# snap-stanford/KGWAS

Measured on AMD Instinct MI355X. Metric: edges aggregated/sec (full fast-mode KG minibatch training; epoch time in config), higher is better.
Workload: dtype f32

## Files before the change

### kgwas_amd/csrc/kgw_dense_linear.h

```cpp
#pragma once

namespace {

constexpr int LBM = 128, LBN = 128, LBK = 32, LPAD = 33;

struct LinArgs {
    const float* X; int64_t ldx;
    const float* W; int64_t ldw;
    const float* bias;
    const float* mask;
    int64_t ldm;
    float* Y; int64_t ldy;
    int64_t rows; int K, N;
    int relu, w_kn;
    const int32_t* rows_dev;
};

__device__ __forceinline__ int64_t lin_rows_eff(const LinArgs& a) {
    if (!a.rows_dev) return a.rows;
    const int64_t r = *a.rows_dev;
    return r < 0 ? 0 : (r < a.rows ? r : a.rows);
}

__device__ __forceinline__ void lin_zero_padding(const LinArgs& a, int64_t rows_eff, int64_t tid, int64_t nthreads) {
// ... 1151 lines not shown
#pragma unroll
            for (int e = 0; e < 16; ++e) acc[t][e] = 0.f;
#pragma unroll
        for (int s_ = 0; s_ < 8; ++s_) {
            const f32x4 u = xa[2 * s_], v = xa[2 * s_ + 1];
            const float h[8] = {kgw_fxor(u.x, sgn), kgw_fxor(u.y, sgn), kgw_fxor(u.z, sgn), kgw_fxor(u.w, sgn),
                                kgw_fxor(v.x, sgn), kgw_fxor(v.y, sgn), kgw_fxor(v.z, sgn), kgw_fxor(v.w, sgn)};
            uint4 p1, p2, p3;
            kgw_split3x8(h, p1, p2, p3);
            const kgw_bf8 hb[3] = {__builtin_bit_cast(kgw_bf8, p1), __builtin_bit_cast(kgw_bf8, p2), __builtin_bit_cast(kgw_bf8, p3)};
            kgw_bf8 wa[3][4];
#pragma unroll
            for (int p = 0; p < 3; ++p)
#pragma unroll
                for (int jt = 0; jt < 4; ++jt) wa[p][jt] = __builtin_bit_cast(kgw_bf8, w2p[((s_ * 3 + p) * 4 + jt) * 64]);
            constexpr int TW[6] = {0, 2, 1, 0, 1, 0}, TH[6] = {2, 0, 1, 1, 0, 0};
#pragma unroll
            for (int t6 = 0; t6 < 6; ++t6)
#pragma unroll
                for (int jt = 0; jt < 4; ++jt)
                    acc[jt] = __builtin_amdgcn_mfma_f32_32x32x16_bf16(wa[TW[t6]][jt], hb[TH[t6]], acc[jt], 0, 0, 0);
            if (s_ == 3) {
                __builtin_amdgcn_sched_barrier(0);
#pragma unroll
                for (int qq = 0; qq < 8; ++qq) xa[qq] = *(const f32x4*)(xn + 4 * qq);
                __builtin_amdgcn_sched_barrier(0);
            }
        }
        if (!live) { mb[0] = 0u; mb[1] = 0u; }
        __builtin_amdgcn_sched_barrier(0);
#pragma unroll
        for (int qq = 8; qq < 16; ++qq) xa[qq] = *(const f32x4*)(xn + 4 * qq);
        __builtin_amdgcn_sched_barrier(0);
#pragma unroll
        for (int hh = 0; hh < 2; ++hh) {
#pragma unroll
            for (int t = 2 * hh; t < 2 * hh + 2; ++t)
#pragma unroll
                for (int g = 0; g < 4; ++g) {
                    const unsigned m4 = mb[t >> 1] >> (((t & 1) << 4) + 4 * g);
                    f32x4 v;
                    v.x = (m4 & 1u) ? kgw_fxor(acc[t][4 * g + 0], sgn) : 0.f; v.y = (m4 & 2u) ? kgw_fxor(acc[t][4 * g + 1], sgn) : 0.f;
                    v.z = (m4 & 4u) ? kgw_fxor(acc[t][4 * g + 2], sgn) : 0.f; v.w = (m4 & 8u) ? kgw_fxor(acc[t][4 * g + 3], sgn) : 0.f;
                    *(f32x4*)(Tw + li * TS2 + (t - 2 * hh) * 32 + 8 * g + 4 * lk) = v;
                    if (a.dZ && row < rows) *(f32x4*)(a.dZ + row * a.ldz + t * 32 + 8 * g + 4 * lk) = v;
                }
            __asm__ volatile("s_waitcnt lgkmcnt(0)" ::: "memory");
            if (PACK) {
                const bool neg = a.flip && ((tile / a.flip) & 1);
#pragma unroll
                for (int it = 0; it < 4; ++it) {
                    const int ntl = it & 1, j = it >> 1;
                    const float* tp = Tw + (16 * j + 8 * lk) * TS2 + 32 * ntl + li;
                    float x[8];
#pragma unroll
                    for (int i = 0; i < 8; ++i) x[i] = neg ? -tp[i * TS2] : tp[i * TS2];
                    uint4 p1, p2, p3;
                    kgw_split3x8(x, p1, p2, p3);
                    uint4* o = a.packed + (((int64_t)tile * 2 + j) * 3 * 4 + (2 * hh + ntl)) * 64 + lane;
                    o[0] = p1; o[4 * 64] = p2; o[8 * 64] = p3;
                }
            }
#pragma unroll
            for (int s2 = 0; s2 < 16; ++s2) {
                const float* tp = Tw + (2 * s2 + lk) * TS2 + li;
#pragma unroll
                for (int t = 0; t < 2; ++t)
                    accw[2 * hh + t] = __builtin_amdgcn_mfma_f32_32x32x2f32(xs[s2], tp[t * 32], accw[2 * hh + t], 0, 0, 0);
            }
            __asm__ volatile("s_waitcnt lgkmcnt(0)" ::: "memory");
        }
        mb[0] = 0u; mb[1] = 0u;
        KGW_MLPB_BITS(mvn, mb)
    }
#undef KGW_MLPB_BITS
    __syncthreads();
    float* R = lds;
#pragma unroll
    for (int t = 0; t < 4; ++t)
#pragma unroll
        for (int e = 0; e < 16; ++e) R[wave * 4096 + (t * 16 + e) * 64 + lane] = accw[t][e];
    __syncthreads();
    for (int f = tid; f < 4096; f += 256)
        a.part[(int64_t)blockIdx.x * 4096 + f] = (R[f] + R[4096 + f]) + (R[2 * 4096 + f] + R[3 * 4096 + f]);
}

__global__ void __launch_bounds__(1024) k_mlp2_bwd_fold(const float* __restrict__ part, int nblk, int K1, float* __restrict__ dW1,
                                                        int64_t ldw, float* __restrict__ db1) {
    __shared__ float sm[1024];
    const int fl = threadIdx.x & 63, g = threadIdx.x >> 6;
    const int f = blockIdx.x * 64 + fl;
    float s4[4] = {0.f, 0.f, 0.f, 0.f};
    int q = 0;
    for (int b = g; b < nblk; b += 16, ++q) s4[q & 3] += part[(int64_t)b * 4096 + f];
    sm[threadIdx.x] = (s4[0] + s4[1]) + (s4[2] + s4[3]);
    __syncthreads();
    if (g == 0) {
        float sv = 0.f;
#pragma unroll
        for (int k = 0; k < 16; k += 4) sv += (sm[k * 64 + fl] + sm[(k + 1) * 64 + fl]) + (sm[(k + 2) * 64 + fl] + sm[(k + 3) * 64 + fl]);
        const int lane = f & 63, e = (f >> 6) & 15, t = f >> 10;
        const int k = (e & 3) + 8 * (e >> 2) + 4 * (lane >> 5), col = 32 * t + (lane & 31);
        if (k < K1) dW1[(int64_t)col * ldw + k] = sv;
        else if (k == K1) db1[col] = sv;
    }
}

template <bool WKN, bool MASK>
__global__ void __launch_bounds__(256) __attribute__((amdgpu_waves_per_eu(2, 2))) k_linear_wreg_half(LinArgs a_) {
    extern __shared__ __attribute__((aligned(16))) float lds[];
    LinArgs a = a_;
    {
        const int64_t re = lin_rows_eff(a_);
        lin_zero_padding(a_, re, (int64_t)blockIdx.x * 256 + threadIdx.x, (int64_t)gridDim.x * 256);
        a.rows = re;
        if ((int64_t)blockIdx.x * 2 * 32 >= re) return;
    }
    float* Wl = lds;
    const int tid = threadIdx.x, lane = tid & 63, wave = tid >> 6;
    const int li = lane & 31, lk = lane >> 5;
    const int64_t tile = (int64_t)blockIdx.x * 2 + (wave >> 1);
    const int t0 = (wave & 1) * 2;
    const int64_t row = tile * 32 + li;
    const bool live = row < a.rows;
    const int64_t rc = live ? row : a.rows - 1;
    f32x4 xa[16];
    {
        const float* xp = a.X + rc * a.ldx + lk * 64;
#pragma unroll
        for (int q = 0; q < 16; ++q) xa[q] = *(const f32x4*)(xp + 4 * q);
    }
    f32x4 mv[2][4];
    if (MASK) {
        const float* mp = a.mask + rc * a.ldm + 4 * lk;
#pragma unroll
        for (int t = 0; t < 2; ++t)
#pragma unroll
            for (int g = 0; g < 4; ++g) mv[t][g] = *(const f32x4*)(mp + (t0 + t) * 32 + 8 * g);
    }
    {
        f32x4 wv[16];
#pragma unroll
        for (int it = 0; it < 16; ++it) {
            const int idx = tid + 256 * it;
            if (!WKN) wv[it] = *(const f32x4*)(a.W + (int64_t)(idx >> 5) * a.ldw + (idx & 31) * 4);
            else wv[it] = *(const f32x4*)(a.W + (int64_t)(idx & 127) * a.ldw + (idx >> 7) * 4);
        }
#pragma unroll
        for (int it = 0; it < 16; ++it) {
            const int idx = tid + 256 * it;
            if (!WKN) {
                *(f32x4*)(Wl + (idx >> 5) * WST + (idx & 31) * 4) = wv[it];
            } else {
                const int k = idx & 127, n4 = (idx >> 7) * 4;
                Wl[(n4 + 0) * WST + k] = wv[it].x; Wl[(n4 + 1) * WST + k] = wv[it].y;
                Wl[(n4 + 2) * WST + k] = wv[it].z; Wl[(n4 + 3) * WST + k] = wv[it].w;
            }
        }
    }
    if (tid < 128) Wl[128 * WST + tid] = a.bias ? a.bias[tid] : 0.f;
    __syncthreads();
    f32x4 bw[2][16];
#pragma unroll
    for (int t = 0; t < 2; ++t)
#pragma unroll
        for (int q = 0; q < 16; ++q) bw[t][q] = *(const f32x4*)(Wl + ((t0 + t) * 32 + li) * WST + lk * 64 + 4 * q);
// ... 135 lines not shown
        static KgwPerDevice attr3_set;
        if (attr3_set.need()) {
            KGW_HIP(hipFuncSetAttribute((const void*)k_mlp2_fwd3, hipFuncAttributeMaxDynamicSharedMemorySize, (int)lds3));
        }
        const int64_t nblk3 = ((rows + 31) / 32 + 7) / 8;
        k_mlp2_fwd3<<<(int)(nblk3 < 256 ? nblk3 : 256), 512, lds3, (hipStream_t)stream_>>>(a);
        KGW_LAUNCH_CHECK();
        return KGW_OK;
    }
    const int64_t nblk = ((rows + 31) / 32 + 3) / 4;
    k_mlp2_fwd<<<(int)(nblk < 256 ? nblk : 256), 256, lds, (hipStream_t)stream_>>>(a);
    KGW_LAUNCH_CHECK();
    return KGW_OK;
}

extern "C" int kgw_mlp2w_fwd(int32_t n_jobs, const float* const* src, const int32_t* const* ids, const int64_t* n_rows,
                             int64_t ldx, const float* W1, int64_t ldw1, const float* b1, const float* W2, int64_t ldw2,
                             const float* b2, float* Xg, float* H1, float* H2, int64_t ldo, kgw_stream_t stream_) {
    if (n_jobs <= 0) return KGW_OK;
    if (n_jobs > 4) return KGW_E_RANGE;
    if (!src || !ids || !n_rows || !W1 || !W2 || !Xg || !H1 || !H2) return KGW_E_NULL;
    if ((ldx & 3) || (ldw1 & 3) || (ldw2 & 3) || (ldo & 3) || !aligned16(W1) || !aligned16(W2) || !aligned16(Xg) || !aligned16(H1) ||
        !aligned16(H2))
        return KGW_E_UNSUPPORTED;
    Mlp2wArgs a{};
    a.n_jobs = n_jobs; a.ldx = ldx;
    a.row0[0] = 0;
    for (int j = 0; j < n_jobs; ++j) {
        if (!src[j] || !ids[j] || n_rows[j] < 0) return KGW_E_NULL;
        if (!aligned16(src[j])) return KGW_E_UNSUPPORTED;
        a.src[j] = src[j]; a.ids[j] = ids[j]; a.row0[j + 1] = a.row0[j] + n_rows[j];
    }
    a.rows = a.row0[n_jobs];
    if (a.rows == 0) return KGW_OK;
    a.W1 = W1; a.ldw1 = ldw1; a.b1 = b1; a.W2 = W2; a.ldw2 = ldw2; a.b2 = b2;
    a.Xg = Xg; a.H1 = H1; a.H2 = H2; a.ldo = ldo;
    const size_t lds = (size_t)(2 * 128 * WST + 256) * sizeof(float);
    static KgwPerDevice attr_once;
    if (attr_once.need()) {
        KGW_HIP(hipFuncSetAttribute((const void*)k_mlp2w_fwd, hipFuncAttributeMaxDynamicSharedMemorySize, (int)lds));
    }
    const int64_t ntiles = (a.rows + 31) / 32;
    k_mlp2w_fwd<<<(unsigned)((ntiles + 1) / 2), 256, lds, (hipStream_t)stream_>>>(a);
    KGW_LAUNCH_CHECK();
    return KGW_OK;
}

extern "C" int64_t kgw_mlp2_bwd_first_workspace_floats(int64_t rows) {
    int64_t nblk = ((rows + 31) / 32 + 3) / 4;
    if (nblk > 256) nblk = 256;
    if (nblk < 1) nblk = 1;
    return nblk * 4096;
}

static int mlp2_bwd_first(const float* dH2, int64_t ldd, const float* W2, int64_t ldw2, const float* H1, int64_t ldh1,
                          const float* X, int64_t ldx, int32_t K1, int64_t rows, const int32_t* rows_dev, float* dW1,
                          int64_t ldw1, float* db1, float* workspace, int64_t workspace_floats, const int32_t* in_ids,
                          float* dZ, int64_t ldz, kgw_stream_t stream_, KgwGradSrc* defer, void* packed = nullptr, int flip = 0) {
    if (!dH2 || !W2 || !H1 || !db1 || !workspace) return KGW_E_NULL;
    if (defer && K1 > 0 && ldw1 != K1) return KGW_E_UNSUPPORTED;
    if (rows <= 0 || K1 < 0) return KGW_E_RANGE;
    if (K1 > 0 && (!X || !dW1)) return KGW_E_NULL;
    if (dZ && ((ldz & 3) || !aligned16(dZ))) return KGW_E_UNSUPPORTED;
    if (K1 > 31 || (ldd & 3) || (ldw2 & 3) || (ldh1 & 3) || !aligned16(dH2) || !aligned16(W2) || !aligned16(H1)) return KGW_E_UNSUPPORTED;
    int64_t nblk = ((rows + 31) / 32 + 3) / 4;
    if (nblk > 256) nblk = 256;
    if (workspace_floats < nblk * 4096) return KGW_E_RANGE;
    Mlp2BwdArgs a{dH2, ldd, W2, ldw2, H1, ldh1, X, ldx, workspace, rows, K1, rows_dev, in_ids, dZ, ldz, (uint4*)packed, flip};
    const size_t lds = (size_t)(128 * WST + 4 * 32 * TST) * sizeof(float);
    static KgwPerDevice attr_once;
    if (attr_once.need()) {
        KGW_HIP(hipFuncSetAttribute((const void*)k_mlp2_bwd_first, hipFuncAttributeMaxDynamicSharedMemorySize, (int)lds));
    }
    hipStream_t st = (hipStream_t)stream_;
    static const bool split3 = !(getenv("KGW_MLP2_SPLIT") && getenv("KGW_MLP2_SPLIT")[0] == '0');
    if (packed && (!split3 || rows_dev || ((uintptr_t)packed & 15))) return KGW_E_UNSUPPORTED;
    if (split3) {
        const size_t lds3 = (size_t)M3_W2_U4 * 16 + (size_t)(4 * 32 * TS2) * sizeof(float);
        static KgwPerDevice attr3_set;
        if (attr3_set.need()) {
            KGW_HIP(hipFuncSetAttribute((const void*)k_mlp2_bwd_first3<false>, hipFuncAttributeMaxDynamicSharedMemorySize, (int)lds3));
            KGW_HIP(hipFuncSetAttribute((const void*)k_mlp2_bwd_first3<true>, hipFuncAttributeMaxDynamicSharedMemorySize, (int)lds3));
        }
        if (packed) k_mlp2_bwd_first3<true><<<(int)nblk, 256, lds3, st>>>(a);
        else k_mlp2_bwd_first3<false><<<(int)nblk, 256, lds3, st>>>(a);
    } else {
        k_mlp2_bwd_first<<<(int)nblk, 256, lds, st>>>(a);
    }
    KGW_LAUNCH_CHECK();
    if (defer) {
        defer[0] = KgwGradSrc{};
        defer[1] = KgwGradSrc{};
        if (K1 > 0) { defer[0].ws = workspace; defer[0].kind = KGW_GRAD_MLP2_W; defer[0].nblk = (int)nblk; defer[0].K1 = K1; }
        defer[1].ws = workspace; defer[1].kind = KGW_GRAD_MLP2_B; defer[1].nblk = (int)nblk; defer[1].K1 = K1;
        return KGW_OK;
    }
    k_mlp2_bwd_fold<<<4096 / 64, 1024, 0, st>>>(workspace, (int)nblk, K1, dW1, ldw1, db1);
    KGW_LAUNCH_CHECK();
    return KGW_OK;
}

extern "C" int kgw_mlp2_bwd_first(const float* dH2, int64_t ldd, const float* W2, int64_t ldw2, const float* H1, int64_t ldh1,
                                  const float* X, int64_t ldx, int32_t K1, int64_t rows, const int32_t* rows_dev, float* dW1,
                                  int64_t ldw1, float* db1, float* workspace, int64_t workspace_floats, const int32_t* in_ids,
                                  float* dZ, int64_t ldz, kgw_stream_t stream_) {
    return mlp2_bwd_first(dH2, ldd, W2, ldw2, H1, ldh1, X, ldx, K1, rows, rows_dev, dW1, ldw1, db1, workspace, workspace_floats,
                          in_ids, dZ, ldz, stream_, nullptr);
}

extern "C" int kgw_mlp2_bwd_first_partial(const float* dH2, int64_t ldd, const float* W2, int64_t ldw2, const float* H1,
                                          int64_t ldh1, const float* X, int64_t ldx, int32_t K1, int64_t rows,
                                          const int32_t* rows_dev, float* dW1, int64_t ldw1, float* db1, float* workspace,
                                          int64_t workspace_floats, const int32_t* in_ids, float* dZ, int64_t ldz, KgwGradSrc* src,
                                          kgw_stream_t stream_) {
    if (!src) return KGW_E_NULL;
    return mlp2_bwd_first(dH2, ldd, W2, ldw2, H1, ldh1, X, ldx, K1, rows, rows_dev, dW1, ldw1, db1, workspace, workspace_floats,
                          in_ids, dZ, ldz, stream_, src);
}

extern "C" int kgw_mlp2_bwd_first_packed(const float* dH2, int64_t ldd, const float* W2, int64_t ldw2, const float* H1,
                                         int64_t ldh1, const float* X, int64_t ldx, int32_t K1, int64_t rows, float* dW1,
                                         int64_t ldw1, float* db1, float* workspace, int64_t workspace_floats,
                                         const int32_t* in_ids, float* dZ, int64_t ldz, void* packed, int32_t flip, KgwGradSrc* src,
                                         kgw_stream_t stream_) {
    if (!packed) return KGW_E_NULL;
    if (flip < 0 || (flip & (flip - 1))) return KGW_E_RANGE;
    return mlp2_bwd_first(dH2, ldd, W2, ldw2, H1, ldh1, X, ldx, K1, rows, nullptr, dW1, ldw1, db1, workspace, workspace_floats,
                          in_ids, dZ, ldz, stream_, src, packed, flip);
}
```

### kgwas_amd/csrc/kgw_gemm3.hip

```cpp
#include "kgw_common.h"
#include "kgw_riders.h"
#include <stdlib.h>

typedef kgw_bf8 g3_bf8;
typedef __attribute__((ext_vector_type(16))) float g3_f16;
typedef __attribute__((ext_vector_type(4))) float g3_f4;
typedef __attribute__((ext_vector_type(4))) unsigned g3_u4;

static constexpr int G3_CH_U4 = 1536;
static constexpr int G3_FLIP = 16;
static int g3_flip() { return G3_FLIP; }
static constexpr int G3_MAX_ITEMS = 512;

template <bool KN>
__global__ void __launch_bounds__(256) k_g3_pack(const float* __restrict__ S, long lds_, int K, long kv, int vec, uint4* __restrict__ out, int flip) {
    const long t = (long)blockIdx.x * 256 + threadIdx.x;
    if (t >= (long)K * 16) return;
    const int lane = (int)(t & 63), nt = (int)((t >> 6) & 3), j = (int)((t >> 8) & 1);
    const long c = t >> 9;
    const int n = 32 * nt + (lane & 31);
    const long k0 = 32 * c + 16 * j + 8 * (lane >> 5);
    float x[8];
    if (KN) {
#pragma unroll
        for (int i = 0; i < 8; ++i) x[i] = k0 + i < kv ? S[(k0 + i) * lds_ + n] : 0.f;
    } else if (vec && k0 + 8 <= kv) {
        const float4 u = *(const float4*)(S + n * lds_ + k0), v = *(const float4*)(S + n * lds_ + k0 + 4);
        x[0] = u.x; x[1] = u.y; x[2] = u.z; x[3] = u.w; x[4] = v.x; x[5] = v.y; x[6] = v.z; x[7] = v.w;
    } else {
#pragma unroll
        for (int i = 0; i < 8; ++i) x[i] = k0 + i < kv ? S[n * lds_ + k0 + i] : 0.f;
    }
    if (flip && ((c / flip) & 1)) {
#pragma unroll
        for (int i = 0; i < 8; ++i) x[i] = -x[i];
    }
    uint4 p1, p2, p3;
    kgw_split3x8(x, p1, p2, p3);
    uint4* o = out + ((c * 2 + j) * 3 * 4 + nt) * 64 + lane;
    o[0] = p1; o[4 * 64] = p2; o[8 * 64] = p3;
}

struct G3Args {
    const float* A; long lda; int M, K;
    const uint4* Bp;
    float* ws;
    int nsplit, n_tiles, per_xcd, flip;
};

struct G3KArgs { G3Args a; G3Riders R; };
template <int MT, int NW = 4, bool IMG = false>
__global__ void __launch_bounds__(64 * NW, (8 / NW) / MT) k_g3_gemm(G3KArgs ka_) {
    const G3Args& a = ka_.a;
    constexpr int NT = 64 * NW, NB = G3_CH_U4 / NT;
    constexpr int NQ = 4 * MT;
    constexpr int AT = 256 * MT;
    __shared__ g3_u4 smB0[G3_CH_U4], smB1[G3_CH_U4];
    __shared__ g3_f4 smA0[IMG ? 1 : NW * AT], smA1[IMG ? 1 : NW * AT];
    const int tid = threadIdx.x, lane = tid & 63, wave = tid >> 6;
    if ((int)blockIdx.x >= a.per_xcd * 8) {
        const char* kseg = (const char*)__builtin_amdgcn_kernarg_segment_ptr();
        const G3Riders* R = (const G3Riders*)(kseg + __builtin_offsetof(G3KArgs, R));
        if (ka_.R.n_blocks) g3_param_riders<NW>(*R, (int)blockIdx.x - a.per_xcd * 8);
        return;
    }
    const int item = (int)(blockIdx.x & 7) * a.per_xcd + (int)(blockIdx.x >> 3);
    if ((int)(blockIdx.x >> 3) >= a.per_xcd || item >= a.n_tiles * a.nsplit) return;
    const int split = item / a.n_tiles, tile = item - split * a.n_tiles;
    const int nch = a.K >> 5;
    const int c0 = (int)((long)nch * split / a.nsplit), c1 = (int)((long)nch * (split + 1) / a.nsplit);
    const int nc = c1 - c0;
    const int row0 = tile * (32 * NW * MT) + wave * (32 * MT);

    const long cstep = a.lda > 0 ? 32 : 1024;
    const float* ap[NQ];
    int aw[NQ];
    if (IMG) {
        int t = row0 >> 5;
        t = t < ((a.M - 1) >> 5) ? t : ((a.M - 1) >> 5);
#pragma unroll
        for (int q = 0; q < NQ; ++q) {
            ap[q] = a.A + (long)t * -a.lda + (long)c0 * 1024 + (q * 64 + lane) * 4;
            aw[q] = 0;
        }
    } else
#pragma unroll
    for (int q = 0; q < NQ; ++q) {
        const int r = 8 * q + (lane >> 3);
        int row = row0 + r;
        row = row < a.M ? row : a.M - 1;
        ap[q] = a.lda ? a.A + (long)row * a.lda + (long)c0 * 32 + (lane & 7) * 4
                      : a.A + ((long)(row >> 5) * nch + c0) * 1024 + (row & 31) * 32 + (lane & 7) * 4;
        aw[q] = wave * AT + r * 8 + ((lane & 7) ^ ((r >> 1) & 7));
    }
    const int m = lane & 31, g = lane >> 5, sw = (m >> 1) & 7;
    const g3_u4* bp = (const g3_u4*)a.Bp + (long)c0 * G3_CH_U4 + tid;

    g3_f4 ra[NQ], rb[NQ];
    g3_u4 bs[NB];
    g3_f16 acc[MT][4];
#pragma unroll
    for (int mt = 0; mt < MT; ++mt)
#pragma unroll
        for (int nt = 0; nt < 4; ++nt)
#pragma unroll
            for (int i = 0; i < 16; ++i) acc[mt][nt][i] = 0.f;

    auto load_a = [&](g3_f4 (&r)[NQ], int c) {
#pragma unroll
        for (int q = 0; q < NQ; ++q) r[q] = __builtin_nontemporal_load((const g3_f4*)(ap[q] + (long)c * cstep));
    };
    auto store_a = [&](const g3_f4 (&r)[NQ], g3_f4* A) {
#pragma unroll
        for (int q = 0; q < NQ; ++q) A[aw[q]] = r[q];
    };
    auto load_b = [&](int c) {
#pragma unroll
        for (int i = 0; i < NB; ++i) bs[i] = bp[(long)c * G3_CH_U4 + i * NT];
    };
    auto store_b = [&](g3_u4* B) {
#pragma unroll
        for (int i = 0; i < NB; ++i) B[tid + i * NT] = bs[i];
    };
    auto compute = [&](const g3_f4* A_, const g3_u4* B_) {
        const g3_u4* B = B_ + lane;
        const g3_f4* A = A_ + wave * AT + m * 8;
#pragma unroll
        for (int j = 0; j < 2; ++j) {
            const int seg = 2 * (2 * j + g);
            g3_bf8 ap_[MT][3];
#pragma unroll
            for (int mt = 0; mt < MT; ++mt) {
                const g3_f4 u = A[mt * 256 + (seg ^ sw)], v = A[mt * 256 + ((seg + 1) ^ sw)];
                const float x[8] = {u[0], u[1], u[2], u[3], v[0], v[1], v[2], v[3]};
                uint4 p1, p2, p3;
                kgw_split3x8(x, p1, p2, p3);
                ap_[mt][0] = __builtin_bit_cast(g3_bf8, p1);
                ap_[mt][1] = __builtin_bit_cast(g3_bf8, p2);
                ap_[mt][2] = __builtin_bit_cast(g3_bf8, p3);
            }
            g3_bf8 b[3][4];
#pragma unroll
            for (int p = 0; p < 3; ++p)
#pragma unroll
                for (int nt = 0; nt < 4; ++nt) b[p][nt] = __builtin_bit_cast(g3_bf8, B[((j * 3 + p) * 4 + nt) * 64]);
            constexpr int TA[6] = {0, 2, 1, 0, 1, 0}, TB[6] = {2, 0, 1, 1, 0, 0};
#pragma unroll
            for (int t = 0; t < 6; ++t)
#pragma unroll
                for (int nt = 0; nt < 4; ++nt)
#pragma unroll
                    for (int mt = 0; mt < MT; ++mt)
                        acc[mt][nt] = __builtin_amdgcn_mfma_f32_32x32x16_bf16(ap_[mt][TA[t]], b[TB[t]][nt], acc[mt][nt], 0, 0, 0);
        }
    };

    auto compute_img = [&](g3_f4 (&r)[NQ], const g3_u4* B_, int cn) {
        const g3_u4* B = B_ + lane;
        g3_bf8 ap_[2][3];
#pragma unroll
        for (int j = 0; j < 2; ++j) {
            const g3_f4 u = r[2 * j], v = r[2 * j + 1];
            const float x[8] = {u[0], u[1], u[2], u[3], v[0], v[1], v[2], v[3]};
            uint4 p1, p2, p3;
            kgw_split3x8(x, p1, p2, p3);
            ap_[j][0] = __builtin_bit_cast(g3_bf8, p1);
            ap_[j][1] = __builtin_bit_cast(g3_bf8, p2);
            ap_[j][2] = __builtin_bit_cast(g3_bf8, p3);
        }
        load_a(r, cn);
#pragma unroll
        for (int j = 0; j < 2; ++j) {
            g3_bf8 b[3][4];
#pragma unroll
            for (int p = 0; p < 3; ++p)
#pragma unroll
                for (int nt = 0; nt < 4; ++nt) b[p][nt] = __builtin_bit_cast(g3_bf8, B[((j * 3 + p) * 4 + nt) * 64]);
            constexpr int TA[6] = {0, 2, 1, 0, 1, 0}, TB[6] = {2, 0, 1, 1, 0, 0};
#pragma unroll
            for (int t = 0; t < 6; ++t)
#pragma unroll
                for (int nt = 0; nt < 4; ++nt)
                    acc[0][nt] = __builtin_amdgcn_mfma_f32_32x32x16_bf16(ap_[j][TA[t]], b[TB[t]][nt], acc[0][nt], 0, 0, 0);
        }
    };

    auto flip = [&]() {
#pragma unroll
        for (int mt = 0; mt < MT; ++mt)
#pragma unroll
            for (int nt = 0; nt < 4; ++nt)
#pragma unroll
                for (int i = 0; i < 16; ++i) acc[mt][nt][i] = -acc[mt][nt][i];
    };
    const int last = nc - 1;
    if constexpr (IMG) {
        static_assert(MT == 1, "the operand image holds 32-row tiles");
        load_a(ra, 0);
        load_b(0);
        store_b(smB0);
        load_a(rb, min(1, last));
        load_b(min(1, last));
        __syncthreads();
        for (int c = 0; c < nc; c += 2) {
            store_b(smB1);
            load_b(min(c + 2, last));
            if (a.flip && c && !((c0 + c) & (a.flip - 1))) flip();
            compute_img(ra, smB0, min(c + 2, last));
            __syncthreads();
            if (c + 1 >= nc) break;
            store_b(smB0);
            load_b(min(c + 3, last));
            if (a.flip && !((c0 + c + 1) & (a.flip - 1))) flip();
            compute_img(rb, smB1, min(c + 3, last));
            __syncthreads();
        }
    } else {
        load_a(ra, 0);
        load_b(0);
        store_a(ra, smA0);
        store_b(smB0);
        load_a(ra, min(1, last));
        load_b(min(1, last));
        __syncthreads();
        for (int c = 0; c < nc; c += 2) {
            load_a(rb, min(c + 2, last));
            store_a(ra, smA1);
            store_b(smB1);
            load_b(min(c + 2, last));
            if (a.flip && c && !((c0 + c) & (a.flip - 1))) flip();
            compute(smA0, smB0);
            __syncthreads();
            if (c + 1 >= nc) break;
            load_a(ra, min(c + 3, last));
            store_a(rb, smA0);
            store_b(smB0);
            load_b(min(c + 3, last));
            if (a.flip && !((c0 + c + 1) & (a.flip - 1))) flip();
            compute(smA1, smB1);
            __syncthreads();
        }
    }

    float* wp = a.ws + ((long)split * a.M) * 128 + m;
    if (a.flip && (((c1 - 1) / a.flip) & 1)) flip();
#pragma unroll
    for (int mt = 0; mt < MT; ++mt)
#pragma unroll
        for (int r = 0; r < 16; ++r) {
            const int row = row0 + 32 * mt + 8 * (r >> 2) + 4 * g + (r & 3);
            if (row < a.M) {
#pragma unroll
                for (int nt = 0; nt < 4; ++nt) wp[(long)row * 128 + 32 * nt] = acc[mt][nt][r];
            }
        }
}

__global__ void __launch_bounds__(256) k_g3_reduce(const float* __restrict__ ws, int nsplit, long M, const float* __restrict__ bias,
                                                   int relu, float* __restrict__ out, long ldo, const int32_t* __restrict__ row_map,
                                                   float* __restrict__ out_rows, long ld_rows, long out_rows_n,
                                                   const int32_t* __restrict__ out_rows_real) {
    const long t = (long)blockIdx.x * 256 + threadIdx.x;
    if (out_rows_real) {
        const long real = *out_rows_real < 0 ? 0 : *out_rows_real;
        const long zr = real + (t >> 5);
        if (zr < out_rows_n) *(float4*)(out_rows + zr * ld_rows + 4 * (t & 31)) = make_float4(0.f, 0.f, 0.f, 0.f);
    }
    if (t >= M * 32) return;
    const long row = t >> 5;
    const int c4 = (int)(t & 31);
    const float4* w = (const float4*)ws + t;
    float4 s = w[0];
    for (int k = 1; k < nsplit; ++k) {
        const float4 v = w[(long)k * M * 32];
        s.x += v.x; s.y += v.y; s.z += v.z; s.w += v.w;
    }
    if (bias) {
        const float4 b = ((const float4*)bias)[c4];
        s.x += b.x; s.y += b.y; s.z += b.z; s.w += b.w;
    }
    if (relu) { s.x = fmaxf(s.x, 0.f); s.y = fmaxf(s.y, 0.f); s.z = fmaxf(s.z, 0.f); s.w = fmaxf(s.w, 0.f); }
    *(float4*)(out + row * ldo + 4 * c4) = s;
    if (row_map) {
        const int l = row_map[row];
        if (l >= 0) *(float4*)(out_rows + (long)l * ld_rows + 4 * c4) = s;
    }
}

__global__ void __launch_bounds__(256) k_g3_reduce_t(const float* __restrict__ ws, int nsplit, long M, float* __restrict__ out, long ldo) {
    __shared__ float tl[32][33];
    const int tid = threadIdx.x;
    const long r0 = (long)blockIdx.x * 32;
    const int cb = blockIdx.y * 32;
    {
        const int r = tid >> 3, c4 = tid & 7;
        float4 s = make_float4(0.f, 0.f, 0.f, 0.f);
        if (r0 + r < M) {
            const float4* w = (const float4*)ws + (r0 + r) * 32 + (cb >> 2) + c4;
            s = w[0];
            for (int k = 1; k < nsplit; ++k) {
                const float4 v = w[(long)k * M * 32];
                s.x += v.x; s.y += v.y; s.z += v.z; s.w += v.w;
            }
        }
        tl[r][4 * c4] = s.x; tl[r][4 * c4 + 1] = s.y; tl[r][4 * c4 + 2] = s.z; tl[r][4 * c4 + 3] = s.w;
    }
    __syncthreads();
    const int r = tid & 31;
    if (r0 + r < M) {
#pragma unroll
        for (int i = 0; i < 4; ++i) {
            const int col = (tid >> 5) + 8 * i;
            out[(long)(cb + col) * ldo + r0 + r] = tl[r][col];
        }
    }
}

static int g3_nw() { return 8; }

static int g3_splits(int64_t M, int64_t K) {
    const int rt = 32 * g3_nw();
    const int64_t tiles = (M + rt - 1) / rt, nch = K / 32;
    int64_t s = (G3_MAX_ITEMS * 4 / g3_nw()) / tiles;
    if (s > nch / 8) s = nch / 8;
    if (s > 16) s = 16;
    if (s < 1) s = 1;
    return (int)s;
}

static bool g3_a_ok(const float* A, int64_t lda, int64_t K) {
    if ((uintptr_t)A & 15) return false;
    if (lda < 0) return !(-lda % 1024) && -lda >= K / 32 * 1024;
    return !(lda & 3);
}

static void g3_gemm_launch(const G3Args& a, const G3Riders& R, int n_riders, hipStream_t st) {
    const int grid = a.per_xcd * 8 + n_riders;
    if (g3_nw() == 8) {
        if (a.lda < 0) k_g3_gemm<1, 8, true><<<grid, 512, 0, st>>>(G3KArgs{a, R});
        else k_g3_gemm<1, 8><<<grid, 512, 0, st>>>(G3KArgs{a, R});
    } else {
        if (a.lda < 0) k_g3_gemm<1, 4, true><<<grid, 256, 0, st>>>(G3KArgs{a, R});
        else k_g3_gemm<1, 4><<<grid, 256, 0, st>>>(G3KArgs{a, R});
    }
}

extern "C" int64_t kgw_gemm3_packed_bytes(int64_t K) { return K > 0 && K % 32 == 0 ? (K / 32) * G3_CH_U4 * 16 : 0; }

extern "C" int64_t kgw_gemm3_workspace_floats(int64_t M, int64_t K) {
    return M > 0 && K > 0 ? (int64_t)g3_splits(M, K) * M * 128 : 0;
}

extern "C" int kgw_gemm3_pack(const float* S, int64_t lds_, int64_t K, int64_t k_valid, int32_t s_is_kn, void* packed,
                              kgw_stream_t stream_) {
    if (!S || !packed) return KGW_E_NULL;
    if (K <= 0 || k_valid < 0 || k_valid > K) return KGW_E_RANGE;
    if (K % 32 || ((uintptr_t)packed & 15)) return KGW_E_UNSUPPORTED;
    hipStream_t st = (hipStream_t)stream_;
    const int64_t nthr = K * 16;
    const int vec = !(lds_ & 3) && !((uintptr_t)S & 15);
    if (s_is_kn) k_g3_pack<true><<<(int)((nthr + 255) / 256), 256, 0, st>>>(S, lds_, (int)K, (long)k_valid, 0, (uint4*)packed, g3_flip());
    else k_g3_pack<false><<<(int)((nthr + 255) / 256), 256, 0, st>>>(S, lds_, (int)K, (long)k_valid, vec, (uint4*)packed, g3_flip());
    KGW_LAUNCH_CHECK();
    return KGW_OK;
}

extern "C" int kgw_gemm3_flip(void) { return g3_flip(); }

extern "C" int kgw_gemm3_partial(const float* A, int64_t lda, int64_t M, int64_t K, const void* packed, float* workspace,
                                 int64_t workspace_floats, float* out, int64_t ldo, KgwGradSrc* src, kgw_stream_t stream_) {
    if (!A || !packed || !workspace || !out || !src) return KGW_E_NULL;
    if (M <= 0 || K <= 0 || M > (1 << 30) || K > (1 << 30)) return KGW_E_RANGE;
    if (K % 32 || M % 32 || ldo != M || !g3_a_ok(A, lda, K) || ((uintptr_t)packed & 15) || ((uintptr_t)workspace & 15))
        return KGW_E_UNSUPPORTED;
    const int ns = g3_splits(M, K);
    if (workspace_floats < (int64_t)ns * M * 128) return KGW_E_RANGE;
    const int rt = 32 * g3_nw();
    const int tiles = (int)((M + rt - 1) / rt);
    const int per_xcd = (tiles * ns + 7) / 8;
    G3Args a{A, (long)lda, (int)M, (int)K, (const uint4*)packed, workspace, ns, tiles, per_xcd, g3_flip()};
    const G3Riders none{};
    g3_gemm_launch(a, none, 0, (hipStream_t)stream_);
    KGW_LAUNCH_CHECK();
    *src = KgwGradSrc{};
    src->ws = workspace; src->kind = KGW_GRAD_G3T; src->nblk = ns; src->M = (int32_t)M; src->N = 128;
    return KGW_OK;
}

static int g3_free_cus(int64_t M, int64_t K) {
    static int n_cu = 0;
    if (!n_cu) {
        int dev = 0;
        hipDeviceProp_t p;
        if (hipGetDevice(&dev) == hipSuccess && hipGetDeviceProperties(&p, dev) == hipSuccess) n_cu = p.multiProcessorCount;
        if (n_cu <= 0) n_cu = 256;
    }
    if (g3_nw() != 8 || M <= 0 || K <= 0) return 0;
    const int ns = g3_splits(M, K);
    const int tiles = (int)((M + 255) / 256);
    const int grid = ((tiles * ns + 7) / 8) * 8;
    int idle = n_cu - grid;
    if (idle > 16) idle = 16;
    return idle >= 8 ? idle : 0;
}

extern "C" int kgw_gemm3_rider_blocks(int64_t M, int64_t K) { return g3_free_cus(M, K); }

static int gemm3_launch(const float* A, int64_t lda, int64_t M, int64_t K, const void* packed, float* workspace,
                        int64_t workspace_floats, const float* bias, int32_t relu, float* out, int64_t ldo, int32_t transpose_out,
                        const int32_t* row_map, float* out_rows, int64_t ld_rows, int64_t out_rows_n, const int32_t* out_rows_real,
                        const G3Riders& R, kgw_stream_t stream_) {
    if (!A || !packed || !workspace || !out) return KGW_E_NULL;
    if (out_rows_real && (!row_map || out_rows_n < 0 || out_rows_n > M)) return KGW_E_RANGE;
    if (M <= 0 || K <= 0 || M > (1 << 30) || K > (1 << 30)) return KGW_E_RANGE;
    if (K % 32 || !g3_a_ok(A, lda, K) || ((uintptr_t)packed & 15) || ((uintptr_t)workspace & 15)) return KGW_E_UNSUPPORTED;
    if (!transpose_out && ((ldo & 3) || ((uintptr_t)out & 15) || (bias && ((uintptr_t)bias & 15)))) return KGW_E_UNSUPPORTED;
    if (transpose_out && (bias || relu || row_map)) return KGW_E_UNSUPPORTED;
    if (row_map && (!out_rows || (ld_rows & 3) || ((uintptr_t)out_rows & 15))) return KGW_E_UNSUPPORTED;
    const int ns = g3_splits(M, K);
    if (workspace_floats < (int64_t)ns * M * 128) return KGW_E_RANGE;
    const int rt = 32 * g3_nw();
    const int tiles = (int)((M + rt - 1) / rt);
    hipStream_t st = (hipStream_t)stream_;
    const int per_xcd = (tiles * ns + 7) / 8;
    G3Args a{A, (long)lda, (int)M, (int)K, (const uint4*)packed, workspace, ns, tiles, per_xcd, g3_flip()};
    g3_gemm_launch(a, R, R.n_blocks, st);
    KGW_LAUNCH_CHECK();
// ... 30 lines not shown
```

Baseline: 1.057 billion.

## Split MLP2 backward first kernel across two half-waves per tile with 512 threads

Adds a new variant of the MLP2 backward first-stage kernel that launches 512 threads per block. Each 32-row tile is processed by two waves, each owning half of the 128 output columns. This halves per-wave accumulator and register pressure and doubles the waves available for latency hiding. The cost is duplicated dH2 row loads and bf16 splitting per wave pair, plus a larger LDS footprint. It is enabled by default and can be turned off with KGW_MLP2_BWD_HALF=0.

```diff
diff --git a/kgwas_amd/csrc/kgw_dense_linear.h b/kgwas_amd/csrc/kgw_dense_linear.h
--- a/kgwas_amd/csrc/kgw_dense_linear.h
+++ b/kgwas_amd/csrc/kgw_dense_linear.h
@@ -1257,6 +1257,200 @@
         for (int e = 0; e < 16; ++e) R[wave * 4096 + (t * 16 + e) * 64 + lane] = accw[t][e];
     __syncthreads();
     for (int f = tid; f < 4096; f += 256)
+        a.part[(int64_t)blockIdx.x * 4096 + f] = (R[f] + R[4096 + f]) + (R[2 * 4096 + f] + R[3 * 4096 + f]);
+}
+
+constexpr int TS3 = 36;
+
+template <bool PACK>
+__global__ void __launch_bounds__(512) __attribute__((amdgpu_waves_per_eu(2, 2))) k_mlp2_bwd_first3h(Mlp2BwdArgs a) {
+    extern __shared__ __attribute__((aligned(16))) float lds[];
+    uint4* W2p = (uint4*)lds;
+    float* Tl = lds + M3_W2_U4 * 4;
+    const int tid = threadIdx.x, lane = tid & 63;
+    const int wv = __builtin_amdgcn_readfirstlane(tid >> 6);
+    const int wave = wv & 3, hh = wv >> 2;
+    const int li = lane & 31, lk = lane >> 5;
+    const unsigned sgn = (li & 1) ? 0x80000000u : 0u;
+    int64_t rows = a.rows;
+    if (a.rows_dev) { const int64_t r = *a.rows_dev; rows = r < 0 ? 0 : (r < a.rows ? r : a.rows); }
+    const int ntiles = (int)((rows + 31) / 32);
+    const int nw = (int)gridDim.x * 4;
+    float* Tw = Tl + wv * 32 * TS3;
+    const int K1 = a.K1;
+    int tile = (int)blockIdx.x * 4 + wave;
+    f32x4 xa[16];
+    int src_cur;
+    f32x4 mv0[2][4];
+    {
+        int64_t r = (int64_t)(tile < ntiles ? tile : ntiles - 1) * 32 + li;
+        if (r >= rows) r = rows - 1;
+        if (r < 0) r = 0;
+        src_cur = a.in_ids ? a.in_ids[r] : 0;
+        const float* xp = a.dH2 + (a.in_ids ? (int64_t)(src_cur < 0 ? 0 : src_cur) : r) * a.ldd + lk * 64;
+        const float* mp = a.H1 + r * a.ldm + 64 * hh + 4 * lk;
+#pragma unroll
+        for (int q = 0; q < 16; ++q) xa[q] = *(const f32x4*)(xp + 4 * q);
+#pragma unroll
+        for (int t_ = 0; t_ < 2; ++t_)
+#pragma unroll
+            for (int g = 0; g < 4; ++g) mv0[t_][g] = *(const f32x4*)(mp + t_ * 32 + 8 * g);
+    }
+    {
+        float xw[4][8];
+#pragma unroll
+        for (int it = 0; it < 4; ++it) {
+            const int idx = tid + 512 * it;
+            const int ln = idx & 63, jt = (idx >> 6) & 3, s_ = idx >> 8;
+            const float* wp = a.W2 + (int64_t)(64 * (ln >> 5) + 8 * s_) * a.ldw + 32 * jt + (ln & 31);
+#pragma unroll
+            for (int i = 0; i < 8; ++i) xw[it][i] = wp[(int64_t)i * a.ldw];
+        }
+#pragma unroll
+        for (int it = 0; it < 4; ++it) {
+            const int idx = tid + 512 * it;
+            const int ln = idx & 63, jt = (idx >> 6) & 3, s_ = idx >> 8;
+            uint4 p1, p2, p3;
+            kgw_split3x8(xw[it], p1, p2, p3);
+            uint4* o = W2p + ((s_ * 3) * 4 + jt) * 64 + ln;
+            o[0] = p1; o[4 * 64] = p2; o[8 * 64] = p3;
+        }
+    }
+    __syncthreads();
+    const uint4* w2p = W2p + 2 * hh * 64 + lane;
+    f32x16 accw[2];
+#pragma unroll
+    for (int t = 0; t < 2; ++t)
+#pragma unroll
+        for (int e = 0; e < 16; ++e) accw[t][e] = 0.f;
+#define KGW_MLPB_BITS(MV, MB)                                                                            \
+    MB = 0u;                                                                                             \
+    _Pragma("unroll") for (int t_ = 1; t_ >= 0; --t_) _Pragma("unroll") for (int g = 3; g >= 0; --g) {  \
+        MB = (MB << 1) | (MV[t_][g].w > 0.f ? 1u : 0u);                                                  \
+        MB = (MB << 1) | (MV[t_][g].z > 0.f ? 1u : 0u);                                                  \
+        MB = (MB << 1) | (MV[t_][g].y > 0.f ? 1u : 0u);                                                  \
+        MB = (MB << 1) | (MV[t_][g].x > 0.f ? 1u : 0u);                                                  \
+    }
+    unsigned mb;
+    KGW_MLPB_BITS(mv0, mb)
+    for (; tile < ntiles; tile += nw) {
+        const int64_t r0 = (int64_t)tile * 32;
+        const int64_t row = r0 + li;
+        const bool live = row < rows && src_cur >= 0;
+        const float* xn;
+        const float* mpn;
+        {
+            int nt = tile + nw;
+            if (nt >= ntiles) nt = ntiles - 1;
+            int64_t r = (int64_t)nt * 32 + li;
+            if (r >= rows) r = rows - 1;
+            src_cur = a.in_ids ? a.in_ids[r] : 0;
+            xn = a.dH2 + (a.in_ids ? (int64_t)(src_cur < 0 ? 0 : src_cur) : r) * a.ldd + lk * 64;
+            mpn = a.H1 + r * a.ldm + 64 * hh + 4 * lk;
+        }
+        float xs[16];
+        if (K1 > 0) {
+            const float* xsp = a.X + (li < K1 ? li : 0);
+#pragma unroll
+            for (int s2 = 0; s2 < 16; ++s2) {
+                const int64_t rr = r0 + 2 * s2 + lk;
+                xs[s2] = xsp[(rr < rows ? rr : rows - 1) * a.ldx];
+            }
+        } else {
+#pragma unroll
+            for (int s2 = 0; s2 < 16; ++s2) xs[s2] = 0.f;
+        }
+#pragma unroll
+        for (int s2 = 0; s2 < 16; ++s2) {
+            const int64_t rr = r0 + 2 * s2 + lk;
+            xs[s2] = rr < rows ? (li < K1 ? xs[s2] : (li == K1 ? 1.f : 0.f)) : 0.f;
+        }
+        f32x16 acc[2];
+#pragma unroll
+        for (int t = 0; t < 2; ++t)
+#pragma unroll
+            for (int e = 0; e < 16; ++e) acc[t][e] = 0.f;
+#pragma unroll
+        for (int s_ = 0; s_ < 8; ++s_) {
+            const f32x4 u = xa[2 * s_], v = xa[2 * s_ + 1];
+            const float h[8] = {kgw_fxor(u.x, sgn), kgw_fxor(u.y, sgn), kgw_fxor(u.z, sgn), kgw_fxor(u.w, sgn),
+                                kgw_fxor(v.x, sgn), kgw_fxor(v.y, sgn), kgw_fxor(v.z, sgn), kgw_fxor(v.w, sgn)};
+            uint4 p1, p2, p3;
+            kgw_split3x8(h, p1, p2, p3);
+            const kgw_bf8 hb[3] = {__builtin_bit_cast(kgw_bf8, p1), __builtin_bit_cast(kgw_bf8, p2), __builtin_bit_cast(kgw_bf8, p3)};
+            kgw_bf8 wa[3][2];
+#pragma unroll
+            for (int p = 0; p < 3; ++p)
+#pragma unroll
+                for (int jt = 0; jt < 2; ++jt) wa[p][jt] = __builtin_bit_cast(kgw_bf8, w2p[((s_ * 3 + p) * 4 + jt) * 64]);
+            constexpr int TW[6] = {0, 2, 1, 0, 1, 0}, TH[6] = {2, 0, 1, 1, 0, 0};
+#pragma unroll
+            for (int t6 = 0; t6 < 6; ++t6)
+#pragma unroll
+                for (int jt = 0; jt < 2; ++jt)
+                    acc[jt] = __builtin_amdgcn_mfma_f32_32x32x16_bf16(wa[TW[t6]][jt], hb[TH[t6]], acc[jt], 0, 0, 0);
+            if (s_ == 3) {
+                __builtin_amdgcn_sched_barrier(0);
+#pragma unroll
+                for (int qq = 0; qq < 8; ++qq) xa[qq] = *(const f32x4*)(xn + 4 * qq);
+                __builtin_amdgcn_sched_barrier(0);
+            }
+        }
+        if (!live) mb = 0u;
+        __builtin_amdgcn_sched_barrier(0);
+        f32x4 mvn[2][4];
+#pragma unroll
+        for (int t_ = 0; t_ < 2; ++t_)
+#pragma unroll
+            for (int g = 0; g < 4; ++g) mvn[t_][g] = *(const f32x4*)(mpn + t_ * 32 + 8 * g);
+        __builtin_amdgcn_sched_barrier(0);
+#pragma unroll
+        for (int qq = 8; qq < 16; ++qq) xa[qq] = *(const f32x4*)(xn + 4 * qq);
+        __builtin_amdgcn_sched_barrier(0);
+#pragma unroll
+        for (int tt = 0; tt < 2; ++tt) {
+            const int t = 2 * hh + tt;
+#pragma unroll
+            for (int g = 0; g < 4; ++g) {
+                const unsigned m4 = mb >> ((tt << 4) + 4 * g);
+                f32x4 v;
+                v.x = (m4 & 1u) ? kgw_fxor(acc[tt][4 * g + 0], sgn) : 0.f; v.y = (m4 & 2u) ? kgw_fxor(acc[tt][4 * g + 1], sgn) : 0.f;
+                v.z = (m4 & 4u) ? kgw_fxor(acc[tt][4 * g + 2], sgn) : 0.f; v.w = (m4 & 8u) ? kgw_fxor(acc[tt][4 * g + 3], sgn) : 0.f;
+                *(f32x4*)(Tw + li * TS3 + 8 * g + 4 * lk) = v;
+                if (a.dZ && row < rows) *(f32x4*)(a.dZ + row * a.ldz + t * 32 + 8 * g + 4 * lk) = v;
+            }
+            __asm__ volatile("s_waitcnt lgkmcnt(0)" ::: "memory");
+            if (PACK) {
+                const bool neg = a.flip && ((tile / a.flip) & 1);
+#pragma unroll
+                for (int j = 0; j < 2; ++j) {
+                    const float* tp = Tw + (16 * j + 8 * lk) * TS3 + li;
+                    float x[8];
+#pragma unroll
+                    for (int i = 0; i < 8; ++i) x[i] = neg ? -tp[i * TS3] : tp[i * TS3];
+                    uint4 p1, p2, p3;
+                    kgw_split3x8(x, p1, p2, p3);
+                    uint4* o = a.packed + (((int64_t)tile * 2 + j) * 3 * 4 + t) * 64 + lane;
+                    o[0] = p1; o[4 * 64] = p2; o[8 * 64] = p3;
+                }
+            }
+#pragma unroll
+            for (int s2 = 0; s2 < 16; ++s2)
+                accw[tt] = __builtin_amdgcn_mfma_f32_32x32x2f32(xs[s2], Tw[(2 * s2 + lk) * TS3 + li], accw[tt], 0, 0, 0);
+            __asm__ volatile("s_waitcnt lgkmcnt(0)" ::: "memory");
+        }
+        __builtin_amdgcn_sched_barrier(0);
+        KGW_MLPB_BITS(mvn, mb)
+    }
+#undef KGW_MLPB_BITS
+    __syncthreads();
+    float* R = lds;
+#pragma unroll
+    for (int tt = 0; tt < 2; ++tt)
+#pragma unroll
+        for (int e = 0; e < 16; ++e) R[wave * 4096 + ((2 * hh + tt) * 16 + e) * 64 + lane] = accw[tt][e];
+    __syncthreads();
+    for (int f = tid; f < 4096; f += 512)
         a.part[(int64_t)blockIdx.x * 4096 + f] = (R[f] + R[4096 + f]) + (R[2 * 4096 + f] + R[3 * 4096 + f]);
 }
 
@@ -1558,7 +1752,17 @@
             KGW_HIP(hipFuncSetAttribute((const void*)k_mlp2_bwd_first3<false>, hipFuncAttributeMaxDynamicSharedMemorySize, (int)lds3));
             KGW_HIP(hipFuncSetAttribute((const void*)k_mlp2_bwd_first3<true>, hipFuncAttributeMaxDynamicSharedMemorySize, (int)lds3));
         }
-        if (packed) k_mlp2_bwd_first3<true><<<(int)nblk, 256, lds3, st>>>(a);
+        const char* half_env = getenv("KGW_MLP2_BWD_HALF");
+        if (!(half_env && half_env[0] == '0')) {
+            const size_t lds3h = (size_t)M3_W2_U4 * 16 + (size_t)(8 * 32 * TS3) * sizeof(float);
+            static KgwPerDevice attr3h_set;
+            if (attr3h_set.need()) {
+                KGW_HIP(hipFuncSetAttribute((const void*)k_mlp2_bwd_first3h<false>, hipFuncAttributeMaxDynamicSharedMemorySize, (int)lds3h));
+                KGW_HIP(hipFuncSetAttribute((const void*)k_mlp2_bwd_first3h<true>, hipFuncAttributeMaxDynamicSharedMemorySize, (int)lds3h));
+            }
+            if (packed) k_mlp2_bwd_first3h<true><<<(int)nblk, 512, lds3h, st>>>(a);
+            else k_mlp2_bwd_first3h<false><<<(int)nblk, 512, lds3h, st>>>(a);
+        } else if (packed) k_mlp2_bwd_first3<true><<<(int)nblk, 256, lds3, st>>>(a);
         else k_mlp2_bwd_first3<false><<<(int)nblk, 256, lds3, st>>>(a);
     } else {
         k_mlp2_bwd_first<<<(int)nblk, 256, lds, st>>>(a);
```

Result: no change. 1.063 billion (median of 6 runs) (+0.6%).

## Add dedicated image-layout GEMM kernel with direct global-to-LDS DMA for B

Applied to the files above, without the earlier changes.

Replaces the templated IMG path with a dedicated 512-thread kernel for the pre-tiled A image. B chunks now go straight from global memory into LDS through global_load_lds_dwordx4 with m0-based addressing, so they no longer pass through registers before a shared store. The kernel waits on a hand-written vmcnt and barrier and prefetches A with nontemporal loads two chunks ahead. It also forces NW=8 for the non-image path, dropping the NW=4 choice, and relies on inline asm waitcnt counts being right.

```diff
diff --git a/kgwas_amd/csrc/kgw_gemm3.hip b/kgwas_amd/csrc/kgw_gemm3.hip
--- a/kgwas_amd/csrc/kgw_gemm3.hip
+++ b/kgwas_amd/csrc/kgw_gemm3.hip
@@ -49,14 +49,14 @@
 };
 
 struct G3KArgs { G3Args a; G3Riders R; };
-template <int MT, int NW = 4, bool IMG = false>
+template <int MT, int NW>
 __global__ void __launch_bounds__(64 * NW, (8 / NW) / MT) k_g3_gemm(G3KArgs ka_) {
     const G3Args& a = ka_.a;
     constexpr int NT = 64 * NW, NB = G3_CH_U4 / NT;
     constexpr int NQ = 4 * MT;
     constexpr int AT = 256 * MT;
     __shared__ g3_u4 smB0[G3_CH_U4], smB1[G3_CH_U4];
-    __shared__ g3_f4 smA0[IMG ? 1 : NW * AT], smA1[IMG ? 1 : NW * AT];
+    __shared__ g3_f4 smA0[NW * AT], smA1[NW * AT];
     const int tid = threadIdx.x, lane = tid & 63, wave = tid >> 6;
     if ((int)blockIdx.x >= a.per_xcd * 8) {
         const char* kseg = (const char*)__builtin_amdgcn_kernarg_segment_ptr();
@@ -75,15 +75,6 @@
     const long cstep = a.lda > 0 ? 32 : 1024;
     const float* ap[NQ];
     int aw[NQ];
-    if (IMG) {
-        int t = row0 >> 5;
-        t = t < ((a.M - 1) >> 5) ? t : ((a.M - 1) >> 5);
-#pragma unroll
-        for (int q = 0; q < NQ; ++q) {
-            ap[q] = a.A + (long)t * -a.lda + (long)c0 * 1024 + (q * 64 + lane) * 4;
-            aw[q] = 0;
-        }
-    } else
 #pragma unroll
     for (int q = 0; q < NQ; ++q) {
         const int r = 8 * q + (lane >> 3);
@@ -155,36 +146,6 @@
         }
     };
 
-    auto compute_img = [&](g3_f4 (&r)[NQ], const g3_u4* B_, int cn) {
-        const g3_u4* B = B_ + lane;
-        g3_bf8 ap_[2][3];
-#pragma unroll
-        for (int j = 0; j < 2; ++j) {
-            const g3_f4 u = r[2 * j], v = r[2 * j + 1];
-            const float x[8] = {u[0], u[1], u[2], u[3], v[0], v[1], v[2], v[3]};
-            uint4 p1, p2, p3;
-            kgw_split3x8(x, p1, p2, p3);
-            ap_[j][0] = __builtin_bit_cast(g3_bf8, p1);
-            ap_[j][1] = __builtin_bit_cast(g3_bf8, p2);
-            ap_[j][2] = __builtin_bit_cast(g3_bf8, p3);
-        }
-        load_a(r, cn);
-#pragma unroll
-        for (int j = 0; j < 2; ++j) {
-            g3_bf8 b[3][4];
-#pragma unroll
-            for (int p = 0; p < 3; ++p)
-#pragma unroll
-                for (int nt = 0; nt < 4; ++nt) b[p][nt] = __builtin_bit_cast(g3_bf8, B[((j * 3 + p) * 4 + nt) * 64]);
-            constexpr int TA[6] = {0, 2, 1, 0, 1, 0}, TB[6] = {2, 0, 1, 1, 0, 0};
-#pragma unroll
-            for (int t = 0; t < 6; ++t)
-#pragma unroll
-                for (int nt = 0; nt < 4; ++nt)
-                    acc[0][nt] = __builtin_amdgcn_mfma_f32_32x32x16_bf16(ap_[j][TA[t]], b[TB[t]][nt], acc[0][nt], 0, 0, 0);
-        }
-    };
-
     auto flip = [&]() {
 #pragma unroll
         for (int mt = 0; mt < MT; ++mt)
@@ -194,52 +155,29 @@
                 for (int i = 0; i < 16; ++i) acc[mt][nt][i] = -acc[mt][nt][i];
     };
     const int last = nc - 1;
-    if constexpr (IMG) {
-        static_assert(MT == 1, "the operand image holds 32-row tiles");
-        load_a(ra, 0);
-        load_b(0);
+    load_a(ra, 0);
+    load_b(0);
+    store_a(ra, smA0);
+    store_b(smB0);
+    load_a(ra, min(1, last));
+    load_b(min(1, last));
+    __syncthreads();
+    for (int c = 0; c < nc; c += 2) {
+        load_a(rb, min(c + 2, last));
+        store_a(ra, smA1);
+        store_b(smB1);
+        load_b(min(c + 2, last));
+        if (a.flip && c && !((c0 + c) & (a.flip - 1))) flip();
+        compute(smA0, smB0);
+        __syncthreads();
+        if (c + 1 >= nc) break;
+        load_a(ra, min(c + 3, last));
+        store_a(rb, smA0);
         store_b(smB0);
-        load_a(rb, min(1, last));
-        load_b(min(1, last));
+        load_b(min(c + 3, last));
+        if (a.flip && !((c0 + c + 1) & (a.flip - 1))) flip();
+        compute(smA1, smB1);
         __syncthreads();
-        for (int c = 0; c < nc; c += 2) {
-            store_b(smB1);
-            load_b(min(c + 2, last));
-            if (a.flip && c && !((c0 + c) & (a.flip - 1))) flip();
-            compute_img(ra, smB0, min(c + 2, last));
-            __syncthreads();
-            if (c + 1 >= nc) break;
-            store_b(smB0);
-            load_b(min(c + 3, last));
-            if (a.flip && !((c0 + c + 1) & (a.flip - 1))) flip();
-            compute_img(rb, smB1, min(c + 3, last));
-            __syncthreads();
-        }
-    } else {
-        load_a(ra, 0);
-        load_b(0);
-        store_a(ra, smA0);
-        store_b(smB0);
-        load_a(ra, min(1, last));
-        load_b(min(1, last));
-        __syncthreads();
-        for (int c = 0; c < nc; c += 2) {
-            load_a(rb, min(c + 2, last));
-            store_a(ra, smA1);
-            store_b(smB1);
-            load_b(min(c + 2, last));
-            if (a.flip && c && !((c0 + c) & (a.flip - 1))) flip();
-            compute(smA0, smB0);
-            __syncthreads();
-            if (c + 1 >= nc) break;
-            load_a(ra, min(c + 3, last));
-            store_a(rb, smA0);
-            store_b(smB0);
-            load_b(min(c + 3, last));
-            if (a.flip && !((c0 + c + 1) & (a.flip - 1))) flip();
-            compute(smA1, smB1);
-            __syncthreads();
-        }
     }
 
     float* wp = a.ws + ((long)split * a.M) * 128 + m;
@@ -254,6 +192,126 @@
                 for (int nt = 0; nt < 4; ++nt) wp[(long)row * 128 + 32 * nt] = acc[mt][nt][r];
             }
         }
+}
+
+static constexpr int G3_SLOT_BYTES = G3_CH_U4 * 16;
+
+__device__ __forceinline__ void g3_dma_3k(const g3_u4* src, unsigned lds) {
+    unsigned keep;
+    asm volatile("s_mov_b32 %0, m0\n\ts_mov_b32 m0, %2\n\ts_nop 0\n\t"
+                 "global_load_lds_dwordx4 %1, off\n\t"
+                 "global_load_lds_dwordx4 %1, off offset:1024\n\t"
+                 "global_load_lds_dwordx4 %1, off offset:2048\n\t"
+                 "s_mov_b32 m0, %0"
+                 : "=&s"(keep) : "v"(src), "s"(lds) : "memory");
+}
+__device__ __forceinline__ void g3_slot_barrier() {
+    asm volatile("s_waitcnt lgkmcnt(0)\n\ts_waitcnt vmcnt(4)\n\ts_barrier" ::: "memory");
+}
+
+__global__ void __launch_bounds__(512, 1) k_g3_gemm_img(G3KArgs ka_) {
+    const G3Args& a = ka_.a;
+    __shared__ g3_u4 smB[2 * G3_CH_U4];
+    const int tid = threadIdx.x, lane = tid & 63, wave = __builtin_amdgcn_readfirstlane(tid >> 6);
+    if ((int)blockIdx.x >= a.per_xcd * 8) {
+        const char* kseg = (const char*)__builtin_amdgcn_kernarg_segment_ptr();
+        const G3Riders* R = (const G3Riders*)(kseg + __builtin_offsetof(G3KArgs, R));
+        if (ka_.R.n_blocks) g3_param_riders<8>(*R, (int)blockIdx.x - a.per_xcd * 8);
+        return;
+    }
+    const int item = (int)(blockIdx.x & 7) * a.per_xcd + (int)(blockIdx.x >> 3);
+    if ((int)(blockIdx.x >> 3) >= a.per_xcd || item >= a.n_tiles * a.nsplit) return;
+    const int split = item / a.n_tiles, tile = item - split * a.n_tiles;
+    const int nch = a.K >> 5;
+    const int c0 = (int)((long)nch * split / a.nsplit), c1 = (int)((long)nch * (split + 1) / a.nsplit);
+    const int nc = c1 - c0, last = nc - 1;
+    const int row0 = tile * 256 + wave * 32;
+    const int m = lane & 31, g = lane >> 5;
+
+    int t = row0 >> 5;
+    t = t < ((a.M - 1) >> 5) ? t : ((a.M - 1) >> 5);
+    const float* ap = a.A + (long)t * -a.lda + (long)c0 * 1024 + lane * 4;
+    const g3_u4* bsrc = (const g3_u4*)a.Bp + (long)c0 * G3_CH_U4 + wave * 192 + lane;
+    const unsigned lds0 = (unsigned)(size_t)(__attribute__((address_space(3))) void*)smB + (unsigned)wave * 3072u;
+
+    g3_f4 ra[4], rb[4];
+    g3_f16 acc[4];
+#pragma unroll
+    for (int nt = 0; nt < 4; ++nt)
+#pragma unroll
+        for (int i = 0; i < 16; ++i) acc[nt][i] = 0.f;
+
+    auto load_a = [&](g3_f4 (&r)[4], int c) {
+#pragma unroll
+        for (int q = 0; q < 4; ++q) r[q] = __builtin_nontemporal_load((const g3_f4*)(ap + (long)c * 1024 + q * 256));
+    };
+    auto dma_b = [&](int c, int slot) {
+        g3_dma_3k(bsrc + (long)c * G3_CH_U4, __builtin_amdgcn_readfirstlane(lds0 + (unsigned)slot * G3_SLOT_BYTES));
+    };
+    auto arrived = [&](g3_f4 (&r)[4]) {
+        asm volatile("" : "+v"(r[0]), "+v"(r[1]), "+v"(r[2]), "+v"(r[3]));
+    };
+    auto split3 = [&](const g3_f4& u, const g3_f4& v, g3_bf8 (&p)[3]) {
+        const float x[8] = {u[0], u[1], u[2], u[3], v[0], v[1], v[2], v[3]};
+        uint4 p1, p2, p3;
+        kgw_split3x8(x, p1, p2, p3);
+        p[0] = __builtin_bit_cast(g3_bf8, p1);
+        p[1] = __builtin_bit_cast(g3_bf8, p2);
+        p[2] = __builtin_bit_cast(g3_bf8, p3);
+    };
+    auto mma = [&](const g3_bf8 (&p)[3], int slot, int j) {
+        const g3_u4* B = smB + slot * G3_CH_U4 + lane;
+        g3_bf8 b[3][4];
+#pragma unroll
+        for (int q = 0; q < 3; ++q)
+#pragma unroll
+            for (int nt = 0; nt < 4; ++nt) b[q][nt] = __builtin_bit_cast(g3_bf8, B[((j * 3 + q) * 4 + nt) * 64]);
+        constexpr int TA[6] = {0, 2, 1, 0, 1, 0}, TB[6] = {2, 0, 1, 1, 0, 0};
+#pragma unroll
+        for (int s = 0; s < 6; ++s)
+#pragma unroll
+            for (int nt = 0; nt < 4; ++nt)
+                acc[nt] = __builtin_amdgcn_mfma_f32_32x32x16_bf16(p[TA[s]], b[TB[s]][nt], acc[nt], 0, 0, 0);
+    };
+    auto flip = [&]() {
+#pragma unroll
+        for (int nt = 0; nt < 4; ++nt)
+#pragma unroll
+            for (int i = 0; i < 16; ++i) acc[nt][i] = -acc[nt][i];
+    };
+
+    load_a(ra, 0);
+    dma_b(0, 0);
+    load_a(rb, min(1, last));
+    g3_slot_barrier();
+    auto interval = [&](g3_f4 (&r)[4], int c) {
+        g3_bf8 p0[3], p1[3];
+        arrived(r);
+        dma_b(min(c + 1, last), (c + 1) & 1);
+        if (a.flip && c && !((c0 + c) & (a.flip - 1))) flip();
+        split3(r[0], r[1], p0);
+        split3(r[2], r[3], p1);
+        load_a(r, min(c + 2, last));
+        mma(p0, c & 1, 0);
+        mma(p1, c & 1, 1);
+        g3_slot_barrier();
+    };
+    for (int c = 0; c < nc; c += 2) {
+        interval(ra, c);
+        if (c + 1 < nc) interval(rb, c + 1);
+    }
+    asm volatile("s_waitcnt vmcnt(0)" ::: "memory");
+
+    float* wp = a.ws + ((long)split * a.M) * 128 + m;
+    if (a.flip && (((c1 - 1) / a.flip) & 1)) flip();
+#pragma unroll
+    for (int r = 0; r < 16; ++r) {
+        const int row = row0 + 8 * (r >> 2) + 4 * g + (r & 3);
+        if (row < a.M) {
+#pragma unroll
+            for (int nt = 0; nt < 4; ++nt) wp[(long)row * 128 + 32 * nt] = acc[nt][r];
+        }
+    }
 }
 
 __global__ void __launch_bounds__(256) k_g3_reduce(const float* __restrict__ ws, int nsplit, long M, const float* __restrict__ bias,
@@ -336,13 +394,8 @@
 
 static void g3_gemm_launch(const G3Args& a, const G3Riders& R, int n_riders, hipStream_t st) {
     const int grid = a.per_xcd * 8 + n_riders;
-    if (g3_nw() == 8) {
-        if (a.lda < 0) k_g3_gemm<1, 8, true><<<grid, 512, 0, st>>>(G3KArgs{a, R});
-        else k_g3_gemm<1, 8><<<grid, 512, 0, st>>>(G3KArgs{a, R});
-    } else {
-        if (a.lda < 0) k_g3_gemm<1, 4, true><<<grid, 256, 0, st>>>(G3KArgs{a, R});
-        else k_g3_gemm<1, 4><<<grid, 256, 0, st>>>(G3KArgs{a, R});
-    }
+    if (a.lda < 0) k_g3_gemm_img<<<grid, 512, 0, st>>>(G3KArgs{a, R});
+    else k_g3_gemm<1, 8><<<grid, 512, 0, st>>>(G3KArgs{a, R});
 }
 
 extern "C" int64_t kgw_gemm3_packed_bytes(int64_t K) { return K > 0 && K % 32 == 0 ? (K / 32) * G3_CH_U4 * 16 : 0; }
```

Measured after the change: 1.051 billion before, 1.053 billion after (median of 6 runs). No clear change (+0.2%).
